# kfirc1503/generative-audio

Measured on AMD Instinct MI355X. Metric: spectrogram-frames/sec, NPPC K=5 FullSubNet+ train step, higher is better.
Workload: dtype bf16

## Files before the change

### generative-audio_amd/csrc/tcn.hip

```cpp
#include <cstdlib>
#include "common.h"
#include "mfma_tile.h"
#include "nppc_hip.h"

namespace {


template <typename T, int EPI>
__global__ __launch_bounds__(256) void gemm_nt_kernel(GemmArgs g) {
  const int ks = g.ksplit > 1 ? g.ksplit : 1;
  const int z = blockIdx.z / ks, ksl = blockIdx.z % ks;
  const T* A = reinterpret_cast<const T*>(g.A) + (size_t)z * g.strideA + (size_t)ksl * g.K;
  const T* B = reinterpret_cast<const T*>(g.B) + (size_t)z * g.strideB + (size_t)ksl * g.K;
  const int lane = threadIdx.x & 63, wave = threadIdx.x >> 6, n = lane & 15, q = lane >> 4;
  const int r0 = blockIdx.x * 128 + wave * 32, c0 = blockIdx.y * 64;
  const T* ap = A + (size_t)(r0 + n) * g.lda + 8 * q;
  const T* bp = B + (size_t)(c0 + n) * g.ldb + 8 * q;
  f32x4 acc[2][4];
  nt_reg_mainloop<T>(acc, g.K / 32, g.lda, g.ldb, [&](int kk) { return ap + 32 * kk; }, [&](int kk) { return bp + 32 * kk; },
                     g.relu_in);

  const NtEpilogue<T, EPI> ep(g, z, blockIdx.x * 128);
  float s1 = 0.f, s2 = 0.f;
#pragma unroll
// ... 535 lines not shown
constexpr int TT_BM = 128, TT_BR = 64;
template <int BN> constexpr int tt_stage_elems() { return TT_BR * (TT_BM + 8) + TT_BR * (BN + 8); }

__device__ __forceinline__ void tn_xcd_remap(unsigned& bx, unsigned& by, unsigned& bz) {
  if (gridDim.z % 8 == 0) {
    const unsigned tiles = gridDim.x * gridDim.y;
    const unsigned lin = bx + gridDim.x * (by + gridDim.y * bz);
    const unsigned xcd = lin & 7, j = lin >> 3;
    bz = xcd + 8 * (j / tiles);
    const unsigned t = j % tiles;
    bx = t % gridDim.x;
    by = t / gridDim.x;
  }
}

template <int BN, bool BLOCKED = false>
__device__ __forceinline__ void tn_tiled_mainloop(f32x4 (&acc)[4][BN / 32], bf16_t* lds, const bf16_t* __restrict__ Ab, long lda,
                                                  const bf16_t* __restrict__ Bb, long ldb, long nstage, long chunk = 0) {
  constexpr int BM = TT_BM, BR = TT_BR, NT = 2 * BM;
  constexpr int RSA = BM + 8, RSB = BN + 8;
  constexpr int WN = BN / 2;
  constexpr int NJ = WN / 16;
  constexpr int STAGE = tt_stage_elems<BN>();
  const int tid = threadIdx.x, lane = tid & 63, wave = tid >> 6, i16 = lane & 15, qq = lane >> 4;
  const int wm = wave >> 1, wn = wave & 1;

  constexpr int ACH = BM / 8, BCH = BN / 8;
  constexpr int NA = BR * ACH / NT, NB = BR * BCH / NT;
  static_assert(NA == 4 && (NB == 4 || NB == 2 || NB == 1), "staging slots are named registers");
  const int arow = tid / ACH, ac = tid % ACH, brow = tid / BCH, bc = tid % BCH;
  constexpr int ASTEP = NT / ACH, BSTEP = NT / BCH;
  const bf16_t* gA = Ab + (long)arow * lda + ac * 8;
  const bf16_t* gB = Bb + (long)brow * ldb + bc * 8;
  const int sA = arow * RSA + ac * 8, sB = BR * RSA + brow * RSB + bc * 8;
  typedef const __attribute__((address_space(1))) u32x4* tn_gvec;
  u32x4 ra0, ra1, ra2, ra3, rb0, rb1 = {}, rb2 = {}, rb3 = {};
#define TN_GLOAD(r0)                                                            \
  ra0 = *(tn_gvec)(gA + ((r0) + 0 * ASTEP) * lda);         \
  ra1 = *(tn_gvec)(gA + ((r0) + 1 * ASTEP) * lda);         \
  ra2 = *(tn_gvec)(gA + ((r0) + 2 * ASTEP) * lda);         \
  ra3 = *(tn_gvec)(gA + ((r0) + 3 * ASTEP) * lda);         \
  rb0 = *(tn_gvec)(gB + ((r0) + 0 * BSTEP) * ldb);         \
  if (NB >= 2) rb1 = *(tn_gvec)(gB + ((r0) + 1 * BSTEP) * ldb); \
  if (NB == 4) {                                                                \
    rb2 = *(tn_gvec)(gB + ((r0) + 2 * BSTEP) * ldb);       \
    rb3 = *(tn_gvec)(gB + ((r0) + 3 * BSTEP) * ldb);       \
  }
#define TN_LSTORE(buf)                                                          \
  *reinterpret_cast<u32x4*>(&lds[(buf) * STAGE + sA + 0 * ASTEP * RSA]) = ra0;             \
  *reinterpret_cast<u32x4*>(&lds[(buf) * STAGE + sA + 1 * ASTEP * RSA]) = ra1;             \
  *reinterpret_cast<u32x4*>(&lds[(buf) * STAGE + sA + 2 * ASTEP * RSA]) = ra2;             \
  *reinterpret_cast<u32x4*>(&lds[(buf) * STAGE + sA + 3 * ASTEP * RSA]) = ra3;             \
  *reinterpret_cast<u32x4*>(&lds[(buf) * STAGE + sB + 0 * BSTEP * RSB]) = rb0;             \
  if (NB >= 2) *reinterpret_cast<u32x4*>(&lds[(buf) * STAGE + sB + 1 * BSTEP * RSB]) = rb1; \
  if (NB == 4) {                                                                \
    *reinterpret_cast<u32x4*>(&lds[(buf) * STAGE + sB + 2 * BSTEP * RSB]) = rb2;           \
    *reinterpret_cast<u32x4*>(&lds[(buf) * STAGE + sB + 3 * BSTEP * RSB]) = rb3;           \
  }
  auto tfrag = [&](const bf16_t* tile, int rs, int r0, int col0) -> bf16x8 {
    const int q4 = i16 >> 2, p4 = i16 & 3;
    const bf16_t* base = tile + (r0 + 8 * qq + q4) * rs + col0 + 4 * p4;
    const s16x4 lo = __builtin_amdgcn_ds_read_tr16_b64_v4i16((__attribute__((address_space(3))) s16x4*)(base));
    const s16x4 hi = __builtin_amdgcn_ds_read_tr16_b64_v4i16((__attribute__((address_space(3))) s16x4*)(base + 4 * rs));
// ... 123 lines not shown
    for (int e = tid; e < BM * BN; e += 256) {
      const int m = e / BN, n = e % BN;
      if (n < nv) dst[(long)(m0 + m) * p.dst_ld + n0 + n] = tile[m * EP + n];
    }
  }
}

__global__ __launch_bounds__(256, 2) void gemm_tn_grouped_kernel(const nppc_tn_problem* __restrict__ table, long R,
                                                                 long chunk, int nwide) {
  __shared__ __attribute__((aligned(16))) bf16_t lds[2 * tt_stage_elems<128>()];
  unsigned bx = blockIdx.x, by = blockIdx.y, bz = blockIdx.z;
  tn_xcd_remap(bx, by, bz);
  const nppc_tn_problem p = table[bz];
  if ((int)by < nwide) tn_grouped_tile<128>(p, lds, (int)bx * TT_BM, (int)by * 128, R / TT_BR, chunk);
  else tn_grouped_tile<64>(p, lds, (int)bx * TT_BM, nwide * 128, R / TT_BR, chunk);
}

}

namespace {
constexpr int DR_BM = 256;

__device__ __forceinline__ int dr_key(int row, int nch) {
  const int k = (row & 3) | (((row >> 3) & 1) << 2);
  return nch >= 8 ? k : (k & (nch - 1));
}
__device__ __forceinline__ int dr_phys(int bytes_in_row, int key, int nch) {
  const int c = bytes_in_row >> 5;
  int pc = c + key;
  if (pc >= nch) pc -= nch;
// ... 289 lines not shown
  return launch_tn(A, lda, B, ldb, C, ldc, M, N, R, ksplit, 1, 0, 0, stream, batch, sA, sB, sC);
}

extern "C" int nppc_gemm_tn_grouped(const nppc_tn_problem* table, int nprob, int M, int N, long R, void* stream) {
  if (!table || nprob < 1 || M <= 0 || N <= 0 || R <= 0) return NPPC_EBADARG;
  if (M % TT_BM || N % 64 || R % TT_BR || nprob > 65535) return NPPC_EUNSUPPORTED;
  const long nstage = R / TT_BR;
  int nblk = 8;
  while (nstage % nblk) --nblk;
  hipLaunchKernelGGL(gemm_tn_grouped_kernel, dim3(M / TT_BM, N / 128 + (N % 128 != 0), nprob), dim3(256), 0, (hipStream_t)stream,
                     table, R, nstage / nblk, N / 128);
  NPPC_CHECK_LAUNCH();
  return NPPC_OK;
}

extern "C" int nppc_gemm_tn_splitk_taps(const void* A, long lda, const void* B, long ldb, float* C, long ldc, int M, int N,
                                        long R, int ksplit, int Wp, int shift_a, void* stream) {
  return launch_tn(A, lda, B, ldb, C, ldc, M, N, R, ksplit, 9, Wp, shift_a, stream);
}
```

### generative-audio_amd/nppc_audio/_hip.py

```python
import ctypes
import os
import threading

import torch

_HERE = os.path.dirname(os.path.abspath(__file__))
LIB_PATH = os.path.join(_HERE, "libnppc_hip.so")

PREC_BF16 = 0
PREC_F32 = 1
_ERR = {1: "bad argument", 2: "kernel launch failed", 3: "unsupported shape/configuration"}

_lib = None

c_p = ctypes.c_void_p
c_i = ctypes.c_int
c_l = ctypes.c_long
c_f = ctypes.c_float


def lib():
    global _lib
    if _lib is None:
        if not os.path.exists(LIB_PATH):
# ... 39 lines not shown
    for A, lda, B, ldb, dst, dst_ld, nvalid, kind in problems:
        assert A.is_cuda and B.is_cuda and dst.is_cuda and A.dtype == B.dtype == torch.bfloat16 and dst.dtype == torch.float32
        assert lda % 8 == 0 and ldb % 8 == 0 and lda >= M and ldb >= N and A.data_ptr() % 16 == 0 and B.data_ptr() % 16 == 0
        assert (R - 1) * lda + M <= A.numel() and (R - 1) * ldb + N <= B.numel() and 0 <= nvalid <= N
        assert kind in (TN_STORE_ASIS, TN_STORE_TRANSPOSED)
        n_rows, n_cols = (M, nvalid) if kind == TN_STORE_ASIS else (nvalid, M)
        assert dst_ld >= n_cols and (n_rows - 1) * dst_ld + n_cols <= dst.numel()
        rows.append([A.data_ptr(), lda, B.data_ptr(), ldb, dst.data_ptr(), dst_ld, nvalid, kind])
    return torch.tensor(rows, dtype=torch.int64).to(problems[0][0].device)


def mid_bwd_part_elems(B, C, Tp, batch):
    n = c_l()
    call("nppc_tcn_mid_bwd_part_elems", B, C, Tp, batch, ctypes.byref(n))
    return n.value


def conv_thin_part_elems():
    n = c_l()
    call("nppc_conv_thin_part_elems", ctypes.byref(n))
    return n.value


def masked_mse_work_elems():
    n = c_l()
    call("nppc_masked_mse_work_elems", ctypes.byref(n))
    return n.value


def crm_mse_work_elems():
# ... 22 lines not shown
    "nppc_lstm2_ws_plan": [I, L, I, I, I, PI, PI],
    "nppc_lstm2_ws_packed_elems": [PL, PL],
    "nppc_lstm2_ws_pack": [P, P, P, P, I, P, P, P],
    "nppc_lstm2_fwd_ws": [I, P, P, P, P, P, P, P, P, P, P, P, P, P, P, P, I, L, I, I, I, P],
    "nppc_lstm2_coop_bwd_packed_elems": [PL],
    "nppc_lstm2_coop_bwd_pack": [P, P, P, P, I, P, P, P],
    "nppc_lstm2_bwd_coop": [P, P, P, P, P, P, P, P, P, P, P, L, P, L, I, I, P],
    "nppc_lstm2_coop_bwd2_packed_elems": [PL],
    "nppc_lstm2_coop_bwd2_pack": [P, P, P, P, I, P, P, P],
    "nppc_lstm2_bwd_coop2": [P, P, P, P, P, P, P, P, P, P, P, L, P, L, I, I, P],
    "nppc_lstm2_bwd_coop2_head": [P, P, P, P, P, P, P, P, P, P, P, P, L, P, L, I, I, P],
    "nppc_lstm2_coop_bwd4_sizes": [L, PL, PL, PL],
    "nppc_lstm2_coop_bwd4_pack": [P, P, P, P, I, P, P, P],
    "nppc_lstm2_bwd_coop4": [P, P, P, P, P, P, P, P, P, P, P, P, P, L, P, L, I, I, P],
    "nppc_head_dy_gather": [P, P, L, I, I, I, I, P],
    "nppc_sb_head_bwd_w": [I, P, P, P, P, L, I, I, I, I, I, P],
    "nppc_lstm2_bwd_packed_elems": [I, I, PL, PL],
    "nppc_lstm2_pack_weights_bwd": [I, P, P, P, P, I, I, P, P, P],
    "nppc_lstm2_bwd": [I, P, P, P, P, P, P, P, P, P, P, L, I, I, I, P],
    "nppc_stft": [P, P, P, P, I, I, I, I, P],
    "nppc_dropband": [P, P, I, I, I, I, I, P],
    "nppc_cirm_build_compress": [P, P, P, P, P, I, I, I, I, F, P],
    "nppc_cirm_decompress_apply_conj": [P, P, P, P, P, P, P, I, I, I, P],
    "nppc_cirm_decompress_apply": [P, P, P, P, P, P, P, I, I, I, P],
    "nppc_istft": [P, P, P, I, I, I, I, I, P],
    "nppc_rowsum": [P, P, L, I, P],
    "nppc_tsse_fwd": [P, P, P, P, P, P, P, P, I, I, I, P, P, P, P, P, P, P, P, P, P, P, P, I, I, I, I, P],
    "nppc_tsse_fwd_maps": [I, P, I, P, P, P, P, P, P, P, I, I, I, P, P, P, P, P, P, L, P, P, P, P, P, P, P, L, I, I, I, I, I, I, P],
    "nppc_tsse_bwd_maps": [I, P, L, P, I, P, P, P, P, I, I, I, P, P, P, L, P, P, P, P, P, P, P, P, P, P, P, P, P, P, P, P, P, P,
                           I, I, I, I, I, I, P],
# ... 1 lines not shown
    "nppc_gemm_nt": [I, I, P, L, L, P, L, L, P, L, L, P, L, P, L, L, P, L, P, L, I, I, I, I, I, I, I, I, I, P],
    "nppc_tcn_mid_bwd_part_elems": [I, I, I, I, PL],
    "nppc_tcn_mid_bwd": [I, P, P, P, P, P, P, P, P, P, P, P, P, P, P, P, P, P, P, P, P, P, P, P, P, P, P, I, I, I, P,
                         I, I, I, I, I, F, L, L, L, I, I, P],
    "nppc_tcn_mid_bwd_finish": [P, L, P, L, I, I, I, P, P, P, P, P, P, P, P, P, P, I, I, L, L, I, I, P],
    "nppc_gemm_nt_tile": [I, I, I, I, PI],
    "nppc_gemm_nt_colsum": [I, I, P, L, L, P, L, L, P, L, L, P, L, P, L, L, I, I, I, I, I, I, I, P, P],
    "nppc_gemm_nt_gn": [I, P, L, L, P, L, L, P, L, L, P, P, L, P, L, L, P, L, D, F, I, I, I, I, I, I, I, P],
    "nppc_tcn_pack_sconv": [I, P, P, P, P, P, P, P, I, I, I, I, I, I, L, L, L, L, P],
    "nppc_gemm_nt_splitk": [I, P, L, P, L, P, L, I, I, L, I, P],
    "nppc_gemm_tn_splitk": [P, L, P, L, P, L, I, I, L, I, P],
    "nppc_gemm_tn_splitk_rowsum": [P, L, P, L, P, L, I, I, L, I, P, P],
    "nppc_gemm_tn_splitk2": [P, L, P, L, I, P, L, I, P, L, I, L, I, P, P],
    "nppc_gemm_tn_splitk_batched": [P, L, L, P, L, L, P, L, L, I, I, L, I, I, P],
    "nppc_gemm_tn_grouped": [P, I, I, I, L, P],
    "nppc_reduce_slabs_t": [P, I, L, L, P, L, I, I, L, L, I, P],
    "nppc_gemm_tn_splitk_taps": [P, L, P, L, P, L, I, I, L, I, I, I, P],
    "nppc_tcn_dwconv": [I, P, P, P, P, P, P, P, P, P, I, I, I, I, I, I, F, L, L, L, I, P],
    "nppc_tcn_gn_apply": [I, P, P, P, P, P, I, I, I, I, I, F, L, L, L, I, P],
    "nppc_pack_matrix": [I, P, P, I, I, I, I, I, P],
    "nppc_pack_matrix_batched": [I, P, P, I, I, I, I, I, I, I, L, L, L, L, P],
    "nppc_subband_mean": [I, P, I, P, I, L, P, P, P, I, I, I, I, I, P],
    "nppc_subband_stage": [I, P, I, P, I, L, P, P, I, I, I, I, I, I, I, I, P],
    "nppc_sb_head": [I, P, P, P, P, L, I, I, I, I, I, P],
    "nppc_gram": [P, P, P, P, P, I, I, L, P],
    "nppc_combine": [P, P, P, P, P, P, P, I, I, L, P],
    "nppc_gs_solve": [P, P, P, I, I, I, P],
    "nppc_gs_bwd_solve": [P, P, P, P, I, I, I, P],
    "nppc_loss_solve": [P, P, P, P, P, P, P, P, P, P, I, I, P],
    "nppc_loss_bwd_coef": [P, P, P, F, F, P, I, I, P],
# ... 188 lines not shown
```

### generative-audio_amd/nppc_audio/engine.py

```python
import ctypes
from types import SimpleNamespace
from typing import NamedTuple

import numpy as np
import torch

from . import _hip as H
from .gemm import gemm_nt, gemm_nt_gn, lstm_wgrad_mode, reduce_slabs, reduce_slabs_t
from .ops_lstm import (PackedLSTM, PackedLSTMBwd, ROW_PAD, WGRAD_SPLITS, bwd_head_fusable, forward_x_ld, lstm2_backward, lstm2_forward,
                       own_workspaces, padded_rows, rows_view, workspace)

TCN_HIDDEN = 512
TCN_DILATIONS = (1, 2, 5, 9, 1, 2, 5, 9)
BRANCHES = ("", "_real", "_imag")
EPI_PLAIN, EPI_PRELU_STATS, EPI_RESIDUAL, EPI_RELU, EPI_PLAIN_F32, EPI_MASK_POS = 0, 1, 2, 3, 4, 5
LSTM_PARAMS = "sb_model.sequence_model."
TSSE_PARAMS = tuple(f"channel_attention.{m}.{leaf}" for m in ("smallConv1d.0", "middleConv1d.0", "largeConv1d.0",
                                                              "feature_concate_fc", "fc1", "fc2") for leaf in ("weight", "bias"))
TCN_MID_GRADS = ("norm2.weight", "norm2.bias", "norm1.weight", "norm1.bias", "depthwise_conv.weight", "depthwise_conv.bias",
                 "prelu1.weight", "prelu2.weight", "conv1x1.bias")
TCN_WGRAD_SPLITS = 8


def rup(a, b):
# ... 409 lines not shown
            (dg2, 0, x_rows, KX, [(q + "bias_ih_l1", 1, I, 1)]),
            (dg2, 0, h1_rows, Hd, [(q + "weight_ih_l1", Hd, 0, Hd)])]
        if Tv > 1:
            jobs += [(dg1, Nseq, h1_rows, Hd, [(q + "weight_hh_l0", Hd, 0, Hd)]),
                     (dg2, Nseq, h2_rows, Hd, [(q + "weight_hh_l1", Hd, 0, Hd)])]
        mode, fold_bias = lstm_wgrad_mode(self.prec, Hd, KX, Tv, WGRAD_SPLITS, guards is not None)
        if mode == "generic":
            return self._lstm_wgrad_generic(jobs, dg1, dg2, Rr, s)
        S = WGRAD_SPLITS
        assert 64 * S <= ROW_PAD
        slab = self._ws("slab", (S * 4 * Hd * max(Hd, KX),), torch.float32)
        if mode == "fused2":
            slab = self._lstm_wgrad_fused2(dg1, dg2, x_rows, h1_rows, guards, Rr, S, s)
        else:
            self._lstm_wgrad_tn(jobs, slab, fold_bias, Rr, S, s)
        if head is not None:
            dyt_rows, O = head
            rows = (Rr + 64 * S - 1) // (64 * S) * (64 * S)
            H.call("nppc_gemm_tn_splitk", h2_rows, Hd, dyt_rows, 16, slab, 64, Hd, 64, rows, S, s)
            reduce_slabs_t(slab, S, slab_stride=Hd * 64, ld=64, dst=self.g("sb_model.fc_output_layer.weight"), dst_ld=Hd, rows=O,
                           ncols=Hd, stream=s)
            H.colsum(self.prec, dyt_rows, self.g("sb_model.fc_output_layer.bias"), Rr, O, 16, 0, 0, 1,
                     lambda n: self._ws("cs_head", (n,), torch.float32), s)

    def _lstm_wgrad_fused2(self, dg1, dg2, x_rows, h1_rows, guards, Rr, S, s):
        Hd, I, KX, K4, q = self.Hd, self.I, self.KX, 4 * self.Hd, LSTM_PARAMS
        (h1_guard, h2_guard), rows = guards, (Rr + 64 * S - 1) // (64 * S) * (64 * S)
        slab = self._ws("slab2", (S * K4 * 2 * Hd,), torch.float32)
        rsum = self._ws("rowsum", (S, K4), torch.float32)
        H.call("nppc_gemm_tn_splitk2", dg1, K4, h1_guard, Hd, Hd, x_rows, KX, KX, slab, Hd + KX, K4, rows, S, None, s)
        self._scatter_slabs(slab, S, K4 * (Hd + KX), Hd + KX, [(q + "weight_hh_l0", Hd, 0, Hd), (q + "weight_ih_l0", I, Hd, I),
# ... 60 lines not shown
                "gradient accumulation over micro-batches); run backward before the next forward")
        if d.get("consumed"):
            raise RuntimeError("direction-net backward called twice for one forward (retain_graph / double backward are "
                               "not supported: the flat gradient buffer is overwritten, not accumulated)")
        d["consumed"] = True
        p = self._backward_plan(d)
        G = self._grad_buffer()
        G.zero_()
        dx, dg1, dg2, head = self._bwd_head_lstm(d, p, dout)
        self._bwd_lstm_wgrad(d, p, G, dg1, dg2, head)
        dpre_fb, Dsb = self._bwd_staging(d, dx)
        w = self._bwd_workspaces(d, p)
        self._bwd_fc(d, p, w, dpre_fb)
        dX0 = self._bwd_tcn(d, p, w, G)
        self._bwd_tsse(d, dX0, dx, Dsb)
        self._bwd_fc_wgrad_join(d, p, w, dpre_fb)
        return G

    def _on_side(self, fn):
        ev = torch.cuda.Event()
        ev.record(torch.cuda.current_stream())
        with torch.cuda.stream(self._side):
            self._side.wait_event(ev)
            fn()

    def _bwd_head_lstm(self, d, p, dout):
        s = H.stream()
        lo, Nseq, Fo, Tv, Hd, O = d["lstm"], d["Nseq"], d["Fo"], d["Tv"], self.Hd, self.O
        gW, gb = self.g("sb_model.fc_output_layer.weight"), self.g("sb_model.fc_output_layer.bias")
        if not p.fused_head:
            dh2 = self._ws("dh2", (Tv, Nseq, Hd))
# ... 17 lines not shown
                             guards=(lo["h1_guard"], lo["h2_guard"]) if "h1_guard" in lo else None)
            if p.early:
                self.grad_range_hook(G, self.fp.off[LSTM_PARAMS + "weight_ih_l0"][0], G.numel())

    def _bwd_staging(self, d, dx):
        B, Tp, ldF = d["B"], d["Tp"], self.ldF
        dpre_fb = self._ws("dpre_fb", (3, B, Tp, ldF), zero=True)
        Dsb = self._ws("Dsb", (B,), torch.float64)
        H.call("nppc_subband_stage_bwd", self.prec, dx, d["x_tm"], d["fb"], d["sbscale"], Dsb, dpre_fb, B, self.F, Tp, d["Tv"], ldF,
               B * Tp * ldF, self.nb, self.G, self.KX, H.stream())
        return dpre_fb, Dsb

    def _bwd_workspaces(self, d, p):
        B, Tp, ldC, R, ws = d["B"], d["Tp"], self.ldC, d["B"] * d["Tp"], self._ws
        w = SimpleNamespace(slab2=None)
        w.tA = ws("tA", (3, max(p.Cr, TCN_HIDDEN, p.Fr), R), zero=True)
        w.tB = ws("tB", (3, max(ldC, TCN_HIDDEN), R), zero=True)
        w.sTA, w.sTB = w.tA.shape[1] * R, w.tB.shape[1] * R
        h2b = ws("h2b", (3, B, Tp, TCN_HIDDEN))
        if p.tn_ok:
            w.dXL = [ws(f"dX_{i}", (3, B, Tp, ldC)) for i in range(9)]
            w.a2L = [ws(f"a2_{i}", (3, B, Tp, TCN_HIDDEN), zero=True) for i in range(8)]
            w.h2L = [ws(f"h2b_{i}", (3, B, Tp, TCN_HIDDEN)) for i in range(8)]
        else:
            w.slab2 = ws("slab2", (3 * p.S2 * max(p.Cr * TCN_HIDDEN, TCN_HIDDEN * ldC, p.Fr * ldC),), torch.float32)
            dXa, dXb = ws("dXa", (3, B, Tp, ldC)), ws("dXb", (3, B, Tp, ldC))
            w.dXL = [dXb if i % 2 else dXa for i in range(9)]
            w.a2L, w.h2L = [d["a2"]] * 8, [h2b] * 8
        w.cpL = list(ws("colpart", (8, 3, R // 128, ldC), torch.float32)) if p.cs_ok else [None] * 8
        return w

    def _fc_wgrad(self, d, p, w, dpre_fb, slab):
        F, ldF, R = self.F, self.ldF, d["B"] * d["Tp"]
        H.colsum(self.prec, dpre_fb, self.g("fb_model.fc_output_layer.bias"), R, F, ldF, R * ldF, self.sP, 3,
                 lambda n: self._ws("cs_fc", (n,), torch.float32), H.stream())
        self._wgrad(d, p, w, "fb_model.fc_output_layer.weight", A=(dpre_fb, F, ldF), rows=(p.Fr, F), B=(d["X"][8], self.ldC),
                    ncols=self.C, slab=slab, relu_b=1)

    def _bwd_fc(self, d, p, w, dpre_fb):
        ldC, ldF, R = self.ldC, self.ldF, d["B"] * d["Tp"]
        if not p.tn_ok:
            self._fc_wgrad(d, p, w, dpre_fb, w.slab2)
        gemm_nt(self.prec, EPI_MASK_POS, A=(dpre_fb, ldF, R * ldF), B=(self.WfcT, ldF, ldC * ldF), C=(w.dXL[8], ldC, R * ldC),
                res=(d["X"][8], ldC, R * ldC), R=R, N=ldC, K=ldF, Tp=d["Tp"], Tv=d["Tv"], Nv=self.C, batch=3, colpart=w.cpL[7],
                stream=H.stream())

    def _tcn_mid_finish(self, d, p, w, Pmid, lo, hi):
        pre, ldC, R = f"fb_model.sequence_model.{lo}.", self.ldC, d["B"] * d["Tp"]
        lay = self.fp.off["fb_model.sequence_model.1.conv1x1.weight"][0] - self.fp.off["fb_model.sequence_model.0.conv1x1.weight"][0]
        H.call("nppc_tcn_mid_bwd_finish", Pmid[lo], Pmid.shape[1], w.cpL[lo], 3 * (R // 128) * ldC, R // 128, ldC, self.C,
               *[self.g(pre + n) for n in TCN_MID_GRADS], self.g(pre + "sconv.bias") if p.cs_ok else None,
               d["B"], TCN_HIDDEN, self.sP, lay, 3, hi - lo, H.stream())

    def _tcn_wgrad_parity(self, d, p, w, i):
        C, ldC, pre = self.C, self.ldC, f"fb_model.sequence_model.{i}."
        self._wgrad(d, p, w, pre + "sconv.weight", A=(w.dXL[i + 1], ldC, ldC), rows=(p.Cr, C), B=(w.a2L[i], TCN_HIDDEN),
# ... 43 lines not shown

    def _bwd_tsse(self, d, dX0, dx, Dsb):
        s, B, T, Tp, F, ldC = H.stream(), d["B"], d["T"], d["Tp"], self.F, self.ldC
        if self.nm == 1:
            H.call("nppc_subband_unfold_bwd", self.prec, dx, d["sbscale"], Dsb, self.mult, dX0[0], ldC, B, F, Tp, d["Tv"], self.nb,
                   self.G, self.KX, s)
        sv = d["tsse_saved"]
        n_ws = ctypes.c_long()
        H.call("nppc_tsse_bwd_ws_elems", 3 * self.nm, B, F, self.ks[0], self.ks[1], self.ks[2], ctypes.byref(n_ws))
        dsg = self._ws("dsg", (n_ws.value,), torch.float32)
        wts = [self.p(n) for n in TSSE_PARAMS if n.endswith(".weight")]
        H.call("nppc_tsse_bwd_maps", self.prec, dX0, B * Tp * ldC, H.ptr_array(d["maps"]), 3 * self.nm, d["rs"], *wts[:3],
               self.ks[0], self.ks[1], self.ks[2], *wts[3:], self.sAtt, sv["ns"], sv["pre"], sv["sq"], sv["h1"], sv["sg"], dsg,
               *[self.g(n) for n in TSSE_PARAMS], B, F, T, self.la, Tp, ldC, s)

    def _bwd_fc_wgrad_join(self, d, p, w, dpre_fb):
        if p.tn_ok:
            self._fc_wgrad(d, p, w, dpre_fb, self._ws("slab_fc", (3 * p.S2 * p.Fr * self.ldC,), torch.float32))
        if self.defer_join:
            self.join_pending = True
            FSNEngine._unjoined[id(self)] = self
        else:
            torch.cuda.current_stream().wait_stream(self._side)

    def side_stream(self):
        return self._side

    def prepack_on_side(self):
        self._on_side(self.pack_weights)
        self.join_pending = True
        FSNEngine._unjoined[id(self)] = self

    def join_side(self):
# ... 10 lines not shown
```

### include/nppc_hip.h

```cpp
#ifndef NPPC_HIP_H
#define NPPC_HIP_H
#ifdef __cplusplus
extern "C" {
#endif

int nppc_stft(const float* wave, float* re, float* im, float* mag , int B, int L, int nfft, int hop,
              void* stream);
int nppc_dropband(const float* in, float* out, int B, int C, int F, int T, int G, void* stream);
int nppc_cirm_build_compress(const float* nr, const float* ni, const float* cr, const float* ci, float* out, int B, int F,
                             int T, int G, float eps, void* stream);
int nppc_cirm_decompress_apply_conj(const float* crm, const float* nr, const float* ni, float* dec ,
                                    float* emag, float* ere, float* eim, int B, int F, int T, void* stream);

int nppc_cirm_decompress_apply(const float* crm, const float* nr, const float* ni, float* dec , float* emag,
                               float* ere, float* eim, int B, int F, int T, void* stream);
int nppc_istft(const float* re, const float* im, float* out, int B, int T, int nfft, int hop, int L, void* stream);

int nppc_rowsum(const float* x, double* sums, long R, int T, void* stream);
int nppc_tsse_fwd_maps(int prec, const float* const* maps, int nmaps, double* rowsum, const float* cw0, const float* cb0,
                       const float* cw1, const float* cb1, const float* cw2, const float* cb2, int ks0, int ks1, int ks2,
                       const float* fcw, const float* fcb, const float* w1, const float* b1, const float* w2, const float* b2, long sW,
                       float* scale, float* ns, float* pre, float* sq, float* h1, float* sg, void* X0, long sY, int B, int C, int T,
                       int look_ahead, int Tp, int ld, void* stream);
int nppc_tsse_bwd_ws_elems(int nmaps, int B, int C, int ks0, int ks1, int ks2, long* elems);
// ... 29 lines not shown
int nppc_gemm_tn_splitk_rowsum(const void* A, long lda, const void* B, long ldb, float* C, long ldc, int M, int N, long R,
                               int ksplit, float* rowsum, void* stream);
int nppc_gemm_tn_splitk2(const void* A, long lda, const void* B1, long ldb1, int N1, const void* B2, long ldb2, int N2, float* C,
                         long ldc, int M, long R, int ksplit, float* rowsum, void* stream);
int nppc_gemm_tn_splitk_batched(const void* A, long lda, long sA, const void* B, long ldb, long sB, float* C, long ldc, long sC,
                                int M, int N, long R, int ksplit, int batch, void* stream);
enum { NPPC_TN_STORE_ASIS = 0, NPPC_TN_STORE_TRANSPOSED = 1 };
typedef struct nppc_tn_problem {
  const void* A; long lda;
  const void* B; long ldb;
  float* dst; long dst_ld;
  long nvalid;
  long kind;
} nppc_tn_problem;
int nppc_gemm_tn_grouped(const nppc_tn_problem* table, int nprob, int M, int N, long R, void* stream);
int nppc_gemm_tn_splitk_taps(const void* A, long lda, const void* B, long ldb, float* C, long ldc, int M, int N, long R,
                             int ksplit, int Wp, int shift_a, void* stream);
int nppc_pack_matrix(int prec, const float* src, void* dst, int N, int K, int Npad, int ldd, int transpose, void* stream);
int nppc_pack_matrix_batched(int prec, const float* src, void* dst, int N, int K, int Npad, int ldd, int transpose, int n_a,
                             int n_b, long src_stride_a, long src_stride_b, long dst_stride_a, long dst_stride_b, void* stream);
int nppc_tcn_dwconv(int prec, const void* in, void* out, const double* st1, double* st2, const float* gamma,
                    const float* beta, const float* wd, const float* bd, const float* slope2, int B, int Cc, int ld, int Tp,
                    int Tv, int dil, float eps, long sAct, long sSt, long sP, int batch, void* stream);
int nppc_tcn_gn_apply(int prec, const void* in, void* out, const double* st, const float* gamma, const float* beta, int B,
                      int Cc, int ld, int Tp, int Tv, float eps, long sAct, long sSt, long sP, int batch, void* stream);
int nppc_tcn_gn_bwd(int prec, const void* dA, const void* y, const double* st, const float* gamma, const float* slope,
                    double* S, void* dpre, float* dgamma, float* dbeta, float* dslope, int B, int Cc, int Tp, int Tv, float eps,
                    long sAct, long sSt, long sP, int batch, void* stream);
int nppc_tcn_dwconv_bwd(int prec, const void* du, const void* y1, const double* st1, const float* gamma, const float* beta,
                        const float* wd, void* dz, float* dwd, float* dbd, int B, int Cc, int Tp, int Tv, int dil, float eps,
// ... 78 lines not shown
int nppc_lstm2_coop_bwd2_pack(const float* w_ih0, const float* w_hh0, const float* w_ih1, const float* w_hh1, int I, void* wb1,
                              void* wb2, void* stream);
int nppc_lstm2_bwd_coop2(const void* g1, const void* g2, const void* c1, const void* c2, const void* dh2, const void* wb1,
                         const void* wb2, void* dx, void* dg1, void* dg2, void* xch, long xch_bytes, unsigned* flags, long N,
                         int Tn, int n_cu, void* stream);
int nppc_lstm2_bwd_coop2_head(const void* g1, const void* g2, const void* c1, const void* c2, const void* dyt, const void* whT,
                              const void* wb1, const void* wb2, void* dx, void* dg1, void* dg2, void* xch, long xch_bytes,
                              unsigned* flags, long N, int Tn, int n_cu, void* stream);
int nppc_lstm2_coop_bwd4_sizes(long N, long* packed_elems, long* xch_bytes, long* flag_words);
int nppc_lstm2_coop_bwd4_pack(const float* w_ih0, const float* w_hh0, const float* w_ih1, const float* w_hh1, int I, void* wb1,
                              void* wb2, void* stream);
int nppc_lstm2_bwd_coop4(const void* g1, const void* g2, const void* c1, const void* c2, const void* dh2, const void* dyt,
                         const void* whT, const void* wb1, const void* wb2, void* dx, void* dg1, void* dg2, void* xch,
                         long xch_bytes, unsigned* flags, long N, int Tn, int n_cu, void* stream);
int nppc_head_dy_gather(const float* dout, void* dyt, long Nseq, int Tn, int la, int O, int Fo, void* stream);
int nppc_sb_head_bwd_w(int prec, const float* dout, const void* h2, float* dWh, float* dbh, long Nseq, int Tn, int la, int Hd,
                       int O, int Fo, void* stream);
int nppc_lstm2_bwd_packed_elems(int I, int H, long* n1, long* n2);
int nppc_lstm2_pack_weights_bwd(int prec, const float* w_ih0, const float* w_hh0, const float* w_ih1, const float* w_hh1,
                                int I, int H, void* wb1, void* wb2, void* stream);
int nppc_lstm2_bwd(int prec, const void* g1, const void* g2, const void* c1, const void* c2, const void* dh2,
                   const void* wb1, const void* wb2, void* dx, void* dg1, void* dg2, long N, int Tn, int I, int H,
                   void* stream);

int nppc_gram(const float* a, const float* b_or_null, const float* gt, const float* pred, double* out, int B, int K,
              long N, void* stream);
int nppc_combine(const float* a, const double* M1, const float* b, const double* M2, const float* gt, const float* pred,
                 float* out, int B, int K, long N, void* stream);
int nppc_gs_solve(const double* G, double* C, double* Ch, int B, int K, int KV, void* stream);
int nppc_gs_bwd_solve(const double* G, const double* P, const double* Ch, double* D, int B, int K, int KV, void* stream);
// ... 355 lines not shown
```

Before: 259,200.

## Add dedicated head wgrad kernel and clipped TN GEMM for fc wgrad on side stream

Adds a dedicated MFMA kernel for the sub-band head weight gradient. It computes partial dW and bias per block of 1024 rows, then runs a small reduction, replacing the split-K GEMM plus slab reduction. The fb fc_output weight gradient now uses a new clipped TN GEMM that applies ReLU to B while loading and writes fp32 directly to the weight gradient without a reduction slab. That GEMM runs on the side stream instead of at the join. Together these remove reduction passes and slab traffic and move work off the critical path, at the cost of more kernel code and changed workspace allocation (tA/tB are now only allocated on the non-tn path).

Measured after the change: 259,200, median of 2. Within noise of the previous version (-0.0%).

```diff
diff --git a/generative-audio_amd/csrc/head_wgrad.hip b/generative-audio_amd/csrc/head_wgrad.hip
--- /dev/null
+++ b/generative-audio_amd/csrc/head_wgrad.hip
@@ -0,0 +1,166 @@
+#include "common.h"
+#include "nppc_hip.h"
+
+namespace {
+
+typedef __attribute__((ext_vector_type(4))) short s16x4;
+typedef __attribute__((ext_vector_type(8))) short s16x8;
+
+constexpr int HW_BR = 32;
+constexpr int HW_ROWS = 1024;
+constexpr int HW_DYS = 16 + 8;
+constexpr int HW_FG = 16;
+
+template <int NJ>
+__global__ __launch_bounds__(256) void head_wgrad_kernel(const bf16_t* __restrict__ h2, const bf16_t* __restrict__ dy,
+                                                         float* __restrict__ part, long R, int Hd, int O) {
+  constexpr int W = 64 * NJ, RS = W + 8, CH = W / 8;
+  constexpr int STAGE = HW_BR * RS + HW_BR * HW_DYS;
+  static_assert(HW_BR * CH == 256 * NJ, "NJ chunks of h2 per thread and stage");
+  __shared__ __attribute__((aligned(16))) bf16_t lds[2 * STAGE];
+  typedef const __attribute__((address_space(1))) u32x4* gvec;
+  const int tid = threadIdx.x, lane = tid & 63, wave = tid >> 6, i16 = lane & 15, qq = lane >> 4;
+  const long r_begin = (long)blockIdx.x * HW_ROWS;
+  const long r_end = r_begin + HW_ROWS < R ? r_begin + HW_ROWS : R;
+  const int col_base = blockIdx.y * W;
+  const int nstage = (int)((r_end - r_begin + HW_BR - 1) / HW_BR);
+  const bool with_bias = blockIdx.y == 0 && wave == 0;
+
+  int hrow[NJ], hoff[NJ], hlds[NJ];
+#pragma unroll
+  for (int i = 0; i < NJ; ++i) {
+    const int idx = tid + 256 * i;
+    hrow[i] = idx / CH;
+    hoff[i] = col_base + (idx % CH) * 8;
+    hlds[i] = hrow[i] * RS + (idx % CH) * 8;
+  }
+  const int drow = tid >> 1, dlds = HW_BR * RS + drow * HW_DYS + (tid & 1) * 8;
+  u32x4 rh[NJ], rd = {};
+  auto gload = [&](int s) {
+    const long r0 = r_begin + (long)s * HW_BR;
+#pragma unroll
+    for (int i = 0; i < NJ; ++i) {
+      const long r = r0 + hrow[i];
+      rh[i] = u32x4{0u, 0u, 0u, 0u};
+      if (r < r_end) rh[i] = *(gvec)(h2 + r * Hd + hoff[i]);
+    }
+    if (tid < 64) {
+      const long r = r0 + drow;
+      rd = u32x4{0u, 0u, 0u, 0u};
+      if (r < r_end) rd = *(gvec)(dy + r * 16 + (tid & 1) * 8);
+    }
+  };
+  auto lstore = [&](int buf) {
+#pragma unroll
+    for (int i = 0; i < NJ; ++i) *reinterpret_cast<u32x4*>(&lds[buf * STAGE + hlds[i]]) = rh[i];
+    if (tid < 64) *reinterpret_cast<u32x4*>(&lds[buf * STAGE + dlds]) = rd;
+  };
+  auto tfrag = [&](const bf16_t* tile, int rs, int col0) -> bf16x8 {
+    const int q4 = i16 >> 2, p4 = i16 & 3;
+    const bf16_t* base = tile + (8 * qq + q4) * rs + col0 + 4 * p4;
+    const s16x4 lo = __builtin_amdgcn_ds_read_tr16_b64_v4i16((__attribute__((address_space(3))) s16x4*)(base));
+    const s16x4 hi = __builtin_amdgcn_ds_read_tr16_b64_v4i16((__attribute__((address_space(3))) s16x4*)(base + 4 * rs));
+    s16x8 v = {lo[0], lo[1], lo[2], lo[3], hi[0], hi[1], hi[2], hi[3]};
+    return __builtin_bit_cast(bf16x8, v);
+  };
+  const short one = 0x3F80;
+  const bf16x8 ones = __builtin_bit_cast(bf16x8, s16x8{one, one, one, one, one, one, one, one});
+
+  f32x4 acc[NJ], racc = {0.f, 0.f, 0.f, 0.f};
+#pragma unroll
+  for (int j = 0; j < NJ; ++j) acc[j] = f32x4{0.f, 0.f, 0.f, 0.f};
+  gload(0);
+  lstore(0);
+  __syncthreads();
+  for (int s = 0; s < nstage; ++s) {
+    const int buf = s & 1;
+    if (s + 1 < nstage) gload(s + 1);
+    const bf16_t* th = lds + buf * STAGE;
+    const bf16x8 a = tfrag(th + HW_BR * RS, HW_DYS, 0);
+#pragma unroll
+    for (int j = 0; j < NJ; ++j) acc[j] = mma16(a, tfrag(th, RS, wave * (16 * NJ) + 16 * j), acc[j]);
+    if (with_bias) racc = mma16(a, ones, racc);
+    if (s + 1 < nstage) lstore(buf ^ 1);
+    __syncthreads();
+  }
+  float* pw = part + (size_t)blockIdx.x * (16 * (size_t)Hd + 16);
+#pragma unroll
+  for (int j = 0; j < NJ; ++j)
+#pragma unroll
+    for (int r = 0; r < 4; ++r) {
+      const int o = 4 * qq + r;
+      if (o < O) pw[(size_t)o * Hd + col_base + wave * (16 * NJ) + 16 * j + i16] = acc[j][r];
+    }
+  if (with_bias && i16 == 0)
+#pragma unroll
+    for (int r = 0; r < 4; ++r)
+      if (4 * qq + r < O) pw[16 * (size_t)Hd + 4 * qq + r] = racc[r];
+}
+
+__global__ __launch_bounds__(64 * HW_FG) void head_wgrad_finish_kernel(const float* __restrict__ part, int nwg, int Hd, int O,
+                                                                       float* __restrict__ dW, float* __restrict__ db) {
+  __shared__ float sm[HW_FG][64];
+  const int el = threadIdx.x & 63, g = threadIdx.x >> 6;
+  const int e = blockIdx.x * 64 + el, nW = O * Hd, nE = nW + O;
+  const size_t PS = 16 * (size_t)Hd + 16;
+  const int per = (nwg + HW_FG - 1) / HW_FG;
+  const int p0 = g * per, p1 = p0 + per < nwg ? p0 + per : nwg;
+  float s = 0.f;
+  if (e < nE) {
+    const float* p = part + (e < nW ? e : 16 * Hd + (e - nW));
+#pragma unroll 8
+    for (int k = p0; k < p1; ++k) s += p[(size_t)k * PS];
+  }
+  sm[g][el] = s;
+  __syncthreads();
+  if (g == 0 && e < nE) {
+    float t = 0.f;
+#pragma unroll
+    for (int k = 0; k < HW_FG; ++k) t += sm[k][el];
+    if (e < nW) dW[e] = t;
+    else db[e - nW] += t;
+  }
+}
+
+int head_wgrad_nj(int Hd) {
+  const int n = Hd / 64;
+  return n % 6 == 0 ? 6 : (n % 3 == 0 ? 3 : (n % 2 == 0 ? 2 : 1));
+}
+
+}
+
+extern "C" {
+
+int nppc_head_wgrad_shape(long R, int Hd, int* rows_per_wg, long* scratch_elems) {
+  if (R <= 0 || Hd <= 0) return NPPC_EBADARG;
+  if (Hd % 64) return NPPC_EUNSUPPORTED;
+  if (rows_per_wg) *rows_per_wg = HW_ROWS;
+  if (scratch_elems) *scratch_elems = ((R + HW_ROWS - 1) / HW_ROWS) * (16 * (long)Hd + 16);
+  return NPPC_OK;
+}
+
+int nppc_head_wgrad(const void* h2_rows, const void* dyt_rows, long R, int Hd, int O, float* dW, float* db, float* scratch,
+                    long scratch_elems, void* stream) {
+  if (!h2_rows || !dyt_rows || !dW || !db || !scratch || R <= 0 || Hd <= 0 || O < 1) return NPPC_EBADARG;
+  if (O > 16 || Hd % 64) return NPPC_EUNSUPPORTED;
+  if (((uintptr_t)h2_rows | (uintptr_t)dyt_rows) % 16) return NPPC_EBADARG;
+  const long nwg = (R + HW_ROWS - 1) / HW_ROWS;
+  if (nwg > 0x7fffffffL || scratch_elems < nwg * (16 * (long)Hd + 16)) return NPPC_EBADARG;
+  hipStream_t s = (hipStream_t)stream;
+  const int nj = head_wgrad_nj(Hd);
+  const dim3 grid((unsigned)nwg, Hd / (64 * nj));
+  const bf16_t* h = (const bf16_t*)h2_rows;
+  const bf16_t* d = (const bf16_t*)dyt_rows;
+  switch (nj) {
+    case 6: hipLaunchKernelGGL(head_wgrad_kernel<6>, grid, dim3(256), 0, s, h, d, scratch, R, Hd, O); break;
+    case 3: hipLaunchKernelGGL(head_wgrad_kernel<3>, grid, dim3(256), 0, s, h, d, scratch, R, Hd, O); break;
+    case 2: hipLaunchKernelGGL(head_wgrad_kernel<2>, grid, dim3(256), 0, s, h, d, scratch, R, Hd, O); break;
+    default: hipLaunchKernelGGL(head_wgrad_kernel<1>, grid, dim3(256), 0, s, h, d, scratch, R, Hd, O); break;
+  }
+  hipLaunchKernelGGL(head_wgrad_finish_kernel, dim3(ceil_div((long)O * Hd + O, 64)), dim3(64 * HW_FG), 0, s, scratch, (int)nwg, Hd,
+                     O, dW, db);
+  NPPC_CHECK_LAUNCH();
+  return NPPC_OK;
+}
+
+}
diff --git a/generative-audio_amd/csrc/tcn.hip b/generative-audio_amd/csrc/tcn.hip
--- a/generative-audio_amd/csrc/tcn.hip
+++ b/generative-audio_amd/csrc/tcn.hip
@@ -573,9 +573,10 @@
   }
 }
 
-template <int BN, bool BLOCKED = false>
+template <int BN, bool BLOCKED = false, bool CLIP = false>
 __device__ __forceinline__ void tn_tiled_mainloop(f32x4 (&acc)[4][BN / 32], bf16_t* lds, const bf16_t* __restrict__ Ab, long lda,
-                                                  const bf16_t* __restrict__ Bb, long ldb, long nstage, long chunk = 0) {
+                                                  const bf16_t* __restrict__ Bb, long ldb, long nstage, long chunk = 0,
+                                                  int a_cols = TT_BM, int relu_b = 0) {
   constexpr int BM = TT_BM, BR = TT_BR, NT = 2 * BM;
   constexpr int RSA = BM + 8, RSB = BN + 8;
   constexpr int WN = BN / 2;
@@ -593,12 +594,19 @@
   const bf16_t* gB = Bb + (long)brow * ldb + bc * 8;
   const int sA = arow * RSA + ac * 8, sB = BR * RSA + brow * RSB + bc * 8;
   typedef const __attribute__((address_space(1))) u32x4* tn_gvec;
-  u32x4 ra0, ra1, ra2, ra3, rb0, rb1 = {}, rb2 = {}, rb3 = {};
+  u32x4 ra0 = {}, ra1 = {}, ra2 = {}, ra3 = {}, rb0, rb1 = {}, rb2 = {}, rb3 = {};
+  const bool a_ok = !CLIP || ac * 8 < a_cols;
+  typedef __attribute__((ext_vector_type(8))) short tn_s16x8;
+  auto relu8 = [](u32x4 v) -> u32x4 {
+    return __builtin_bit_cast(u32x4, __builtin_elementwise_max(__builtin_bit_cast(tn_s16x8, v), tn_s16x8{0, 0, 0, 0, 0, 0, 0, 0}));
+  };
 #define TN_GLOAD(r0)                                                            \
-  ra0 = *(tn_gvec)(gA + ((r0) + 0 * ASTEP) * lda);         \
-  ra1 = *(tn_gvec)(gA + ((r0) + 1 * ASTEP) * lda);         \
-  ra2 = *(tn_gvec)(gA + ((r0) + 2 * ASTEP) * lda);         \
-  ra3 = *(tn_gvec)(gA + ((r0) + 3 * ASTEP) * lda);         \
+  if (a_ok) {                                                                   \
+    ra0 = *(tn_gvec)(gA + ((r0) + 0 * ASTEP) * lda);       \
+    ra1 = *(tn_gvec)(gA + ((r0) + 1 * ASTEP) * lda);       \
+    ra2 = *(tn_gvec)(gA + ((r0) + 2 * ASTEP) * lda);       \
+    ra3 = *(tn_gvec)(gA + ((r0) + 3 * ASTEP) * lda);       \
+  }                                                                             \
   rb0 = *(tn_gvec)(gB + ((r0) + 0 * BSTEP) * ldb);         \
   if (NB >= 2) rb1 = *(tn_gvec)(gB + ((r0) + 1 * BSTEP) * ldb); \
   if (NB == 4) {                                                                \
@@ -606,6 +614,12 @@
     rb3 = *(tn_gvec)(gB + ((r0) + 3 * BSTEP) * ldb);       \
   }
 #define TN_LSTORE(buf)                                                          \
+  if (CLIP && relu_b) {                                                         \
+    rb0 = relu8(rb0);                                                           \
+    rb1 = relu8(rb1);                                                           \
+    rb2 = relu8(rb2);                                                           \
+    rb3 = relu8(rb3);                                                           \
+  }                                                                             \
   *reinterpret_cast<u32x4*>(&lds[(buf) * STAGE + sA + 0 * ASTEP * RSA]) = ra0;             \
   *reinterpret_cast<u32x4*>(&lds[(buf) * STAGE + sA + 1 * ASTEP * RSA]) = ra1;             \
   *reinterpret_cast<u32x4*>(&lds[(buf) * STAGE + sA + 2 * ASTEP * RSA]) = ra2;             \
@@ -759,6 +773,46 @@
   const nppc_tn_problem p = table[bz];
   if ((int)by < nwide) tn_grouped_tile<128>(p, lds, (int)bx * TT_BM, (int)by * 128, R / TT_BR, chunk);
   else tn_grouped_tile<64>(p, lds, (int)bx * TT_BM, nwide * 128, R / TT_BR, chunk);
+}
+
+template <int BN>
+__device__ __forceinline__ void tn_clip_tile(bf16_t* lds, const bf16_t* __restrict__ A, long lda, const bf16_t* __restrict__ B, long ldb,
+                                             float* __restrict__ dst, long dst_ld, int m0, int n0, int Mv, int Nv, long nstage,
+                                             long chunk, int relu_b) {
+  constexpr int BM = TT_BM, WN = BN / 2, NJ = WN / 16;
+  constexpr int EP = BN + 1;
+  static_assert(BM * EP * 4 <= 2 * tt_stage_elems<BN>() * 2, "the fp32 tile fits into the operand buffers");
+  const int tid = threadIdx.x, lane = tid & 63, wave = tid >> 6, i16 = lane & 15, qq = lane >> 4;
+  const int wm = wave >> 1, wn = wave & 1;
+  f32x4 acc[4][NJ];
+  tn_tiled_mainloop<BN, true, true>(acc, lds, A + m0, lda, B + n0, ldb, nstage, chunk, Mv - m0, relu_b);
+  float* tile = reinterpret_cast<float*>(lds);
+#pragma unroll
+  for (int i = 0; i < 4; ++i)
+#pragma unroll
+    for (int j = 0; j < NJ; ++j)
+#pragma unroll
+      for (int r = 0; r < 4; ++r) tile[(wm * 64 + 16 * i + 4 * qq + r) * EP + wn * WN + 16 * j + i16] = acc[i][j][r];
+  __syncthreads();
+  const int mv = Mv - m0, nv = Nv - n0;
+  for (int e = tid; e < BM * BN; e += 256) {
+    const int m = e / BN, n = e % BN;
+    if (m < mv && n < nv) dst[(long)(m0 + m) * dst_ld + n0 + n] = tile[m * EP + n];
+  }
+}
+
+__global__ __launch_bounds__(256, 2) void gemm_tn_clip_kernel(const bf16_t* __restrict__ A, long lda, long sA,
+                                                              const bf16_t* __restrict__ B, long ldb, long sB,
+                                                              float* __restrict__ dst, long dst_ld, long sDst, int Mv, int Nv,
+                                                              long R, long chunk, int nwide, int relu_b) {
+  __shared__ __attribute__((aligned(16))) bf16_t lds[2 * tt_stage_elems<128>()];
+  const unsigned z = blockIdx.z;
+  A += (size_t)z * sA;
+  B += (size_t)z * sB;
+  dst += (size_t)z * sDst;
+  const int m0 = (int)blockIdx.x * TT_BM;
+  if ((int)blockIdx.y < nwide) tn_clip_tile<128>(lds, A, lda, B, ldb, dst, dst_ld, m0, (int)blockIdx.y * 128, Mv, Nv, R / TT_BR, chunk, relu_b);
+  else tn_clip_tile<64>(lds, A, lda, B, ldb, dst, dst_ld, m0, nwide * 128, Mv, Nv, R / TT_BR, chunk, relu_b);
 }
 
 }
@@ -1078,6 +1132,21 @@
   return NPPC_OK;
 }
 
+extern "C" int nppc_gemm_tn_clip(const void* A, long lda, long sA, const void* B, long ldb, long sB, float* dst, long dst_ld,
+                                 long sDst, int Mv, int Nv, long R, int relu_b, int batch, void* stream) {
+  if (!A || !B || !dst || Mv <= 0 || Nv <= 0 || R <= 0 || batch < 1 || Mv > lda || Nv > ldb || dst_ld < Nv) return NPPC_EBADARG;
+  if (lda % 8 || ldb % 64 || R % TT_BR || sA % 8 || sB % 8 || batch > 65535 || ((uintptr_t)A | (uintptr_t)B) % 16)
+    return NPPC_EUNSUPPORTED;
+  const long nstage = R / TT_BR;
+  int nblk = 8;
+  while (nstage % nblk) --nblk;
+  hipLaunchKernelGGL(gemm_tn_clip_kernel, dim3((Mv + TT_BM - 1) / TT_BM, ldb / 128 + (ldb % 128 != 0), batch), dim3(256), 0,
+                     (hipStream_t)stream, (const bf16_t*)A, lda, sA, (const bf16_t*)B, ldb, sB, dst, dst_ld, sDst, Mv, Nv, R,
+                     nstage / nblk, (int)(ldb / 128), relu_b);
+  NPPC_CHECK_LAUNCH();
+  return NPPC_OK;
+}
+
 extern "C" int nppc_gemm_tn_splitk_taps(const void* A, long lda, const void* B, long ldb, float* C, long ldc, int M, int N,
                                         long R, int ksplit, int Wp, int shift_a, void* stream) {
   return launch_tn(A, lda, B, ldb, C, ldc, M, N, R, ksplit, 9, Wp, shift_a, stream);
diff --git a/generative-audio_amd/nppc_audio/_hip.py b/generative-audio_amd/nppc_audio/_hip.py
--- a/generative-audio_amd/nppc_audio/_hip.py
+++ b/generative-audio_amd/nppc_audio/_hip.py
@@ -77,6 +77,12 @@
     n = c_l()
     call("nppc_tcn_mid_bwd_part_elems", B, C, Tp, batch, ctypes.byref(n))
     return n.value
+
+
+def head_wgrad_shape(R, Hd):
+    rows, n = c_i(), c_l()
+    call("nppc_head_wgrad_shape", R, Hd, ctypes.byref(rows), ctypes.byref(n))
+    return rows.value, n.value
 
 
 def conv_thin_part_elems():
@@ -129,6 +135,8 @@
     "nppc_lstm2_coop_bwd4_pack": [P, P, P, P, I, P, P, P],
     "nppc_lstm2_bwd_coop4": [P, P, P, P, P, P, P, P, P, P, P, P, P, L, P, L, I, I, P],
     "nppc_head_dy_gather": [P, P, L, I, I, I, I, P],
+    "nppc_head_wgrad_shape": [L, I, PI, PL],
+    "nppc_head_wgrad": [P, P, L, I, I, P, P, P, L, P],
     "nppc_sb_head_bwd_w": [I, P, P, P, P, L, I, I, I, I, I, P],
     "nppc_lstm2_bwd_packed_elems": [I, I, PL, PL],
     "nppc_lstm2_pack_weights_bwd": [I, P, P, P, P, I, I, P, P, P],
@@ -160,6 +168,7 @@
     "nppc_gemm_tn_splitk2": [P, L, P, L, I, P, L, I, P, L, I, L, I, P, P],
     "nppc_gemm_tn_splitk_batched": [P, L, L, P, L, L, P, L, L, I, I, L, I, I, P],
     "nppc_gemm_tn_grouped": [P, I, I, I, L, P],
+    "nppc_gemm_tn_clip": [P, L, L, P, L, L, P, L, L, I, I, L, I, I, P],
     "nppc_reduce_slabs_t": [P, I, L, L, P, L, I, I, L, L, I, P],
     "nppc_gemm_tn_splitk_taps": [P, L, P, L, P, L, I, I, L, I, I, I, P],
     "nppc_tcn_dwconv": [I, P, P, P, P, P, P, P, P, P, I, I, I, I, I, I, F, L, L, L, I, P],
diff --git a/generative-audio_amd/nppc_audio/engine.py b/generative-audio_amd/nppc_audio/engine.py
--- a/generative-audio_amd/nppc_audio/engine.py
+++ b/generative-audio_amd/nppc_audio/engine.py
@@ -447,7 +447,12 @@
             slab = self._lstm_wgrad_fused2(dg1, dg2, x_rows, h1_rows, guards, Rr, S, s)
         else:
             self._lstm_wgrad_tn(jobs, slab, fold_bias, Rr, S, s)
-        if head is not None:
+        if head is not None and head[1] <= 16 and Hd % 64 == 0:
+            dyt_rows, O = head
+            part = self._ws("head_part", (H.head_wgrad_shape(Rr, Hd)[1],), torch.float32)
+            H.call("nppc_head_wgrad", h2_rows, dyt_rows, Rr, Hd, O, self.g("sb_model.fc_output_layer.weight"),
+                   self.g("sb_model.fc_output_layer.bias"), part, part.numel(), s)
+        elif head is not None:
             dyt_rows, O = head
             rows = (Rr + 64 * S - 1) // (64 * S) * (64 * S)
             H.call("nppc_gemm_tn_splitk", h2_rows, Hd, dyt_rows, 16, slab, 64, Hd, 64, rows, S, s)
@@ -538,7 +543,7 @@
         self._bwd_fc(d, p, w, dpre_fb)
         dX0 = self._bwd_tcn(d, p, w, G)
         self._bwd_tsse(d, dX0, dx, Dsb)
-        self._bwd_fc_wgrad_join(d, p, w, dpre_fb)
+        self._bwd_join()
         return G
 
     def _on_side(self, fn):
@@ -586,15 +591,15 @@
     def _bwd_workspaces(self, d, p):
         B, Tp, ldC, R, ws = d["B"], d["Tp"], self.ldC, d["B"] * d["Tp"], self._ws
         w = SimpleNamespace(slab2=None)
-        w.tA = ws("tA", (3, max(p.Cr, TCN_HIDDEN, p.Fr), R), zero=True)
-        w.tB = ws("tB", (3, max(ldC, TCN_HIDDEN), R), zero=True)
-        w.sTA, w.sTB = w.tA.shape[1] * R, w.tB.shape[1] * R
         h2b = ws("h2b", (3, B, Tp, TCN_HIDDEN))
         if p.tn_ok:
             w.dXL = [ws(f"dX_{i}", (3, B, Tp, ldC)) for i in range(9)]
             w.a2L = [ws(f"a2_{i}", (3, B, Tp, TCN_HIDDEN), zero=True) for i in range(8)]
             w.h2L = [ws(f"h2b_{i}", (3, B, Tp, TCN_HIDDEN)) for i in range(8)]
         else:
+            w.tA = ws("tA", (3, max(p.Cr, TCN_HIDDEN, p.Fr), R), zero=True)
+            w.tB = ws("tB", (3, max(ldC, TCN_HIDDEN), R), zero=True)
+            w.sTA, w.sTB = w.tA.shape[1] * R, w.tB.shape[1] * R
             w.slab2 = ws("slab2", (3 * p.S2 * max(p.Cr * TCN_HIDDEN, TCN_HIDDEN * ldC, p.Fr * ldC),), torch.float32)
             dXa, dXb = ws("dXa", (3, B, Tp, ldC)), ws("dXb", (3, B, Tp, ldC))
             w.dXL = [dXb if i % 2 else dXa for i in range(9)]
@@ -609,9 +614,18 @@
         self._wgrad(d, p, w, "fb_model.fc_output_layer.weight", A=(dpre_fb, F, ldF), rows=(p.Fr, F), B=(d["X"][8], self.ldC),
                     ncols=self.C, slab=slab, relu_b=1)
 
+    def _fc_wgrad_tn(self, d, dpre_fb):
+        F, ldF, C, ldC, R, s = self.F, self.ldF, self.C, self.ldC, d["B"] * d["Tp"], H.stream()
+        H.colsum(self.prec, dpre_fb, self.g("fb_model.fc_output_layer.bias"), R, F, ldF, R * ldF, self.sP, 3,
+                 lambda n: self._ws("cs_fc", (n,), torch.float32), s)
+        H.call("nppc_gemm_tn_clip", dpre_fb, ldF, R * ldF, d["X"][8], ldC, R * ldC, self.g("fb_model.fc_output_layer.weight"), C,
+               self.sP, F, C, R, 1, 3, s)
+
     def _bwd_fc(self, d, p, w, dpre_fb):
         ldC, ldF, R = self.ldC, self.ldF, d["B"] * d["Tp"]
-        if not p.tn_ok:
+        if p.tn_ok:
+            self._on_side(lambda: self._fc_wgrad_tn(d, dpre_fb))
+        else:
             self._fc_wgrad(d, p, w, dpre_fb, w.slab2)
         gemm_nt(self.prec, EPI_MASK_POS, A=(dpre_fb, ldF, R * ldF), B=(self.WfcT, ldF, ldC * ldF), C=(w.dXL[8], ldC, R * ldC),
                 res=(d["X"][8], ldC, R * ldC), R=R, N=ldC, K=ldF, Tp=d["Tp"], Tv=d["Tv"], Nv=self.C, batch=3, colpart=w.cpL[7],
@@ -685,9 +699,7 @@
                self.ks[0], self.ks[1], self.ks[2], *wts[3:], self.sAtt, sv["ns"], sv["pre"], sv["sq"], sv["h1"], sv["sg"], dsg,
                *[self.g(n) for n in TSSE_PARAMS], B, F, T, self.la, Tp, ldC, s)
 
-    def _bwd_fc_wgrad_join(self, d, p, w, dpre_fb):
-        if p.tn_ok:
-            self._fc_wgrad(d, p, w, dpre_fb, self._ws("slab_fc", (3 * p.S2 * p.Fr * self.ldC,), torch.float32))
+    def _bwd_join(self):
         if self.defer_join:
             self.join_pending = True
             FSNEngine._unjoined[id(self)] = self
diff --git a/include/nppc_hip.h b/include/nppc_hip.h
--- a/include/nppc_hip.h
+++ b/include/nppc_hip.h
@@ -67,6 +67,8 @@
   long kind;
 } nppc_tn_problem;
 int nppc_gemm_tn_grouped(const nppc_tn_problem* table, int nprob, int M, int N, long R, void* stream);
+int nppc_gemm_tn_clip(const void* A, long lda, long sA, const void* B, long ldb, long sB, float* dst, long dst_ld, long sDst,
+                      int Mv, int Nv, long R, int relu_b, int batch, void* stream);
 int nppc_gemm_tn_splitk_taps(const void* A, long lda, const void* B, long ldb, float* C, long ldc, int M, int N, long R,
                              int ksplit, int Wp, int shift_a, void* stream);
 int nppc_pack_matrix(int prec, const float* src, void* dst, int N, int K, int Npad, int ldd, int transpose, void* stream);
@@ -175,6 +177,9 @@
                          const void* whT, const void* wb1, const void* wb2, void* dx, void* dg1, void* dg2, void* xch,
                          long xch_bytes, unsigned* flags, long N, int Tn, int n_cu, void* stream);
 int nppc_head_dy_gather(const float* dout, void* dyt, long Nseq, int Tn, int la, int O, int Fo, void* stream);
+int nppc_head_wgrad_shape(long R, int Hd, int* rows_per_wg, long* scratch_elems);
+int nppc_head_wgrad(const void* h2_rows, const void* dyt_rows, long R, int Hd, int O, float* dW, float* db, float* scratch,
+                    long scratch_elems, void* stream);
 int nppc_sb_head_bwd_w(int prec, const float* dout, const void* h2, float* dWh, float* dbh, long Nseq, int Tn, int la, int Hd,
                        int O, int Fo, void* stream);
 int nppc_lstm2_bwd_packed_elems(int I, int H, long* n1, long* n2);
```
